# ZAX130/SmileCode

Measured on AMD Instinct MI355X. Metric: volume-pairs/sec (160x192x160) fwd+bwd, higher is better.
Workload: dtype f32; 1 GPU; ModeT 160x192x160 fp32, batch=1/GPU, full train step NCC+Grad3d fwd+bwd+Adam-amsgrad; global_batch=1, parallelism=dp1, allreduce=one flat all-reduce after backward

## Files before the change

smilecode_amd/csrc/conv3d_bf16.hip:

```cpp
#include "common.h"
#include "step_ctx.h"
#include "conv3d_internal.h"
#include <mutex>
#include <vector>

namespace {

typedef __attribute__((ext_vector_type(8))) __bf16 bf16x8;
typedef float f32x4 __attribute__((ext_vector_type(4)));
constexpr int NTHR = 256;
constexpr int TX = 16, HX = TX + 2;

__device__ __forceinline__ unsigned pack_bf16x2(float a, float b) {
  const __bf16 x = (__bf16)a, y = (__bf16)b;
  return (unsigned)__builtin_bit_cast(unsigned short, x) | ((unsigned)__builtin_bit_cast(unsigned short, y) << 16);
}
__device__ __forceinline__ unsigned short to_bf16(float a) {
  const __bf16 x = (__bf16)a;
  return __builtin_bit_cast(unsigned short, x);
}
__device__ __forceinline__ float bf16_to_f32(unsigned short u) { return __uint_as_float((unsigned)u << 16); }
__device__ __forceinline__ void split3(float x, unsigned short& hi, unsigned short& mid, unsigned short& lo) {
  hi = to_bf16(x);
  const float r1 = x - bf16_to_f32(hi);
// ... 494 lines not shown
        float4* slot = reinterpret_cast<float4*>(red + (U * 3 * NTB + n) * 256) + lane;
        float4 v = make_float4(accb[n][0], accb[n][1], accb[n][2], accb[n][3]);
        if (w4 > 0) { const float4 o = *slot; v.x += o.x; v.y += o.y; v.z += o.z; v.w += o.w; }
        *slot = v;
      }
    }
  }
  __syncthreads();
  float* out = part + ((size_t)blockIdx.x * gridDim.y + blockIdx.y) * RED_FL;
  for (int i = tid; i < RED_FL; i += NTHR) out[i] = red[i];
}

__host__ __device__ inline int colsum_rg(int gx) { return gx >= 512 ? 16 : (gx >= 256 ? 8 : (gx >= 128 ? 4 : (gx >= 64 ? 2 : 1))); }
__host__ __device__ inline int colsum_blocks(int64_t row_fl, int gx) { return (int)cdiv64(row_fl / 4, 256 / colsum_rg(gx)); }
__device__ __forceinline__ void wgrad_bf16_colsum_body(const float* __restrict__ part, float* __restrict__ red, int gx,
                                                       int64_t row_fl, int blk, double (*sm)[4]) {
  const int RG = colsum_rg(gx), QPB = 256 / RG;
  const int q = threadIdx.x % QPB, rg = threadIdx.x / QPB;
  const int64_t j = ((int64_t)blk * QPB + q) * 4;
  double a0 = 0.0, a1 = 0.0, a2 = 0.0, a3 = 0.0;
  if (j < row_fl) {
    const float* base = part + j;
    int g = rg;
    for (; g + 7 * RG < gx; g += 8 * RG) {
      float4 r[8];
#pragma unroll
      for (int u = 0; u < 8; ++u) r[u] = *reinterpret_cast<const float4*>(base + (int64_t)(g + RG * u) * row_fl);
#pragma unroll
      for (int u = 0; u < 8; ++u) asm volatile("" : "+v"(r[u].x), "+v"(r[u].y), "+v"(r[u].z), "+v"(r[u].w));
#pragma unroll
      for (int u = 0; u < 8; ++u) { a0 += (double)r[u].x; a1 += (double)r[u].y; a2 += (double)r[u].z; a3 += (double)r[u].w; }
    }
    {
      float4 r[8];
#pragma unroll
      for (int u = 0; u < 8; ++u) r[u] = *reinterpret_cast<const float4*>(base + (int64_t)(g + RG * u < gx ? g + RG * u : 0) * row_fl);
#pragma unroll
      for (int u = 0; u < 8; ++u) asm volatile("" : "+v"(r[u].x), "+v"(r[u].y), "+v"(r[u].z), "+v"(r[u].w));
#pragma unroll
      for (int u = 0; u < 8; ++u) {
        const bool in = g + RG * u < gx;
        a0 += in ? (double)r[u].x : 0.0; a1 += in ? (double)r[u].y : 0.0; a2 += in ? (double)r[u].z : 0.0; a3 += in ? (double)r[u].w : 0.0;
      }
    }
  }
  if (RG > 1) {
    sm[threadIdx.x][0] = a0; sm[threadIdx.x][1] = a1; sm[threadIdx.x][2] = a2; sm[threadIdx.x][3] = a3;
    __syncthreads();
    if (rg == 0) {
      for (int k = 1; k < RG; ++k) { a0 += sm[k * QPB + q][0]; a1 += sm[k * QPB + q][1]; a2 += sm[k * QPB + q][2]; a3 += sm[k * QPB + q][3]; }
    }
  }
  if (rg == 0 && j < row_fl) *reinterpret_cast<float4*>(red + j) = make_float4((float)a0, (float)a1, (float)a2, (float)a3);
}
__global__ __launch_bounds__(256) void wgrad_bf16_colsum_kernel(const float* __restrict__ part, float* __restrict__ red,
                                                                int gx, int64_t row_fl) {
  __shared__ double sm[256][4];
  wgrad_bf16_colsum_body(part, red, gx, row_fl, blockIdx.x, sm);
}

__device__ __forceinline__ void wgrad_bf16_reduce_body(const float* __restrict__ part, float* __restrict__ dw,
                                                       float* __restrict__ dbias, int Cin, int Cout, int CIB, int U, int NTB,
                                                       int gx, int gy, int n_coblk, int blk, int layout = 0) {
  const int nW = Cout * Cin * 27;
  const int i = blk * 256 + threadIdx.x;
  if (i >= nW + Cout) return;
  if (layout == 1) {
    const int RED_FL = (U * 2 + 1) * 256;
    int co, slot, m, q = 0;
    if (i < nW) {
      const int tap = i % 27, ci = (i / 27) % Cin;
      co = i / (27 * Cin);
      const int combo = tap / 3, dx = tap % 3;
      const int gl = CIB == 8 ? combo / 2 : combo / 4;
      m = CIB == 8 ? (combo % 2) * 8 + ci : (combo % 4) * 4 + ci;
      slot = gl * 2 + (dx == 2 ? 1 : 0);
      q = dx == 0 ? 1 : 0;
    } else {
      co = i - nW; slot = U * 2; m = 0;
    }
    const int n = q * 8 + co, lane = (m / 4) * 16 + n, reg = m % 4;
    const size_t off = (size_t)slot * 256 + lane * 4 + reg;
    double a = 0.0;
    for (int g = 0; g < gx; ++g) a += (double)part[(size_t)g * RED_FL + off];
    if (i < nW) dw[i] = (float)a;
    else if (dbias) dbias[co] = (float)a;
    return;
  }
  if (layout == 2) {
    const int NQ = CIB, MT = U, NT = NTB;
    const int RED_FL = (MT + 1) * NT * 256;
    int co, by_ci = 0, mt, c = 0, e = 0;
    if (i < nW) {
      const int tap = i % 27, ci = (i / 27) % Cin;
      co = i / (27 * Cin);
      by_ci = ci / (4 * NQ);
      const int q = (tap / 3) * NQ + (ci % (4 * NQ)) / 4;
      mt = (q >> 2) * 3 + tap % 3; c = q & 3; e = ci & 3;
    } else {
      co = i - nW; mt = MT;
    }
    const int cob = co / (16 * NT), nt = (co / 16) % NT, j = co % 16;
    const size_t off = (size_t)(by_ci * n_coblk + cob) * RED_FL + (size_t)(mt * NT + nt) * 256 + (c * 16 + j) * 4 + e;
    double a = 0.0;
    for (int g = 0; g < gx; ++g) a += (double)part[(size_t)g * gy * RED_FL + off];
    if (i < nW) dw[i] = (float)a;
    else if (dbias) dbias[co] = (float)a;
    return;
  }
  const int SLOTS = U * 3 + 1, RED_FL = SLOTS * NTB * 256;
  const int GPB = CIB == 16 ? 9 : (CIB == 8 ? 5 : 3);
  int co, slot, m, chunk;
  if (i < nW) {
    const int tap = i % 27, ci = (i / 27) % Cin;
    co = i / (27 * Cin);
    const int combo = tap / 3, dx = tap % 3;
    int gl;
    if (CIB == 16) { gl = combo; m = ci % 16; }
    else if (CIB == 8) { gl = combo / 2; m = (combo % 2) * 8 + ci; }
    else { gl = combo / 4; m = (combo % 4) * 4 + ci; }
    const int gg = (CIB == 16 ? (ci / 16) * GPB : 0) + gl;
    chunk = gg / U;
    slot = (gg % U) * 3 + dx;
  } else {
    co = i - nW; chunk = 0; slot = U * 3; m = 0;
  }
  const int nbg = co / 16, yb = nbg / NTB, nb = nbg % NTB, n = co % 16;
  const int lane = (m / 4) * 16 + n, reg = m % 4;
  const size_t off = (size_t)(chunk * n_coblk + yb) * RED_FL + (size_t)(slot * NTB + nb) * 256 + lane * 4 + reg;
  double a = 0.0;
  for (int g = 0; g < gx; ++g) a += (double)part[(size_t)g * gy * RED_FL + off];
  if (i < nW) dw[i] = (float)a;
  else if (dbias) dbias[co] = (float)a;
}
__global__ __launch_bounds__(256) void wgrad_bf16_reduce_kernel(const float* __restrict__ part, float* __restrict__ dw,
                                                                float* __restrict__ dbias, int Cin, int Cout, int CIB, int U,
                                                                int NTB, int gx, int gy, int n_coblk, int layout) {
  wgrad_bf16_reduce_body(part, dw, dbias, Cin, Cout, CIB, U, NTB, gx, gy, n_coblk, blockIdx.x, layout);
}

constexpr int BRED_MAX_JOBS = 24;
struct BRedTable { BRedJob job[BRED_MAX_JOBS]; int first[BRED_MAX_JOBS + 1]; int n; };
__global__ __launch_bounds__(256) void wgrad_bf16_colsum_many_kernel(const BRedTable t) {
  __shared__ double sm[256][4];
  int j = 0;
  while (j + 1 < t.n && (int)blockIdx.x >= t.first[j + 1]) ++j;
  const BRedJob& J = t.job[j];
  wgrad_bf16_colsum_body(J.part, J.red, J.gx, J.row_fl, blockIdx.x - t.first[j], sm);
}
__global__ __launch_bounds__(256) void wgrad_bf16_reduce_many_kernel(const BRedTable t) {
  int j = 0;
  while (j + 1 < t.n && (int)blockIdx.x >= t.first[j + 1]) ++j;
  const BRedJob& J = t.job[j];
  wgrad_bf16_reduce_body(J.red, J.dw, J.dbias, J.Cin, J.Cout, J.cib, J.u, J.ntb, 1, J.gy, J.n_coblk, blockIdx.x - t.first[j], J.layout);
}

struct WgBf16Plan { int cib, u, ntb, tz, ty, n_chunk, n_coblk, gy, gx, ntiles, tiles_x, tiles_y, tiles_z, red_fl; };
inline WgBf16Plan plan_wgrad_bf16(int B, int D, int H, int W, int Cin, int Cout) {
  WgBf16Plan p;
  if (Cin <= 4) { p.cib = 4; p.u = 3; p.ntb = 1; p.tz = 4; p.ty = 8; }
  else if (Cin <= 8) { p.cib = 8; p.u = 5; p.ntb = 1; p.tz = 4; p.ty = 8; }
  else if (Cout <= 16) { p.cib = 16; p.u = 9; p.ntb = 1; p.tz = 2; p.ty = 8; }
  else { p.cib = 16; p.u = 3; p.ntb = 2; p.tz = 2; p.ty = 4; }
  const int gpb = p.cib == 16 ? 9 : (p.cib == 8 ? 5 : 3);
  const int nblk = p.cib == 16 ? cdiv(Cin, 16) : 1;
  p.n_chunk = nblk * gpb / p.u;
  p.n_coblk = cdiv(Cout, p.ntb * 16);
  p.gy = p.n_chunk * p.n_coblk;
  p.tiles_x = cdiv(W, WTX); p.tiles_y = cdiv(H, p.ty); p.tiles_z = cdiv(D, p.tz);
  p.ntiles = B * p.tiles_x * p.tiles_y * p.tiles_z;
  int gx = (256 * 2) / p.gy;
  if (gx < 1) gx = 1;
  if (gx > p.ntiles) gx = p.ntiles;
  p.gx = gx;
  p.red_fl = (p.u * 3 + 1) * p.ntb * 256;
  return p;
}

struct Bf16Plan { int tz, ty, ck, nt, nstage, cinp, coutp, ksteps; };
inline int round_up_i(int a, int b) { return (a + b - 1) / b * b; }
inline Bf16Plan plan_tiled(int64_t V, int Cin, int Cout, int sp) {
  Bf16Plan p;
  p.cinp = round_up_i(Cin, 8);
  p.ck = (sp == 1 && p.cinp % 32 == 0) ? 32 : (p.cinp % 16 == 0 ? 16 : 8);
  p.nstage = p.cinp / p.ck;
  p.nt = Cout <= 16 ? 1 : 2;
  p.coutp = round_up_i(Cout, p.nt * 16);
  p.ksteps = (27 * p.ck + 31) / 32;
  if (V >= 60000) { p.tz = (sp == 3 && p.ck == 16) ? 2 : 4; p.ty = 8; }
  else { p.tz = 2; p.ty = 4; }
  return p;
}
inline int tiled_tiles_per_sample(int D, int H, int W, const Bf16Plan& p) { return cdiv(W, TX) * cdiv(H, p.ty) * cdiv(D, p.tz); }

inline size_t bf16_wpk_elems(int Cin, int Cout) {
  return (size_t)28 * round_up_i(Cin, 32) * round_up_i(Cout, 32) + 1024;
}

inline void launch_shift(bool x_bf16, const void* x, const float* w, const float* bias, float* shift, int B, int D, int H, int W,
                         int Cin, int Cout, hipStream_t s) {
  if (x_bf16) hipLaunchKernelGGL(conv_shift_bf16_kernel<true>, dim3(cdiv(B * Cout, 4)), dim3(256), 0, s, x, w, bias, shift, B, D, H, W, Cin, Cout);
  else hipLaunchKernelGGL(conv_shift_bf16_kernel<false>, dim3(cdiv(B * Cout, 4)), dim3(256), 0, s, x, w, bias, shift, B, D, H, W, Cin, Cout);
}

template <bool IN_BF16, bool OUT_BF16, bool STATS, int SP>
int launch_tiled(modet_step_ctx* step, const void* x, const float* w, const float* bias, void* y, void* ws, float* stats, int B,
                 int D, int H, int W, int Cin, int Cout, int mode, hipStream_t s) {
  const Bf16Plan p = plan_tiled((int64_t)D * H * W, Cin, Cout, SP);
  const unsigned short* wpk = prepacked_bf16_or_record(step, PackBKey{w, Cin, Cout, p.coutp, p.ck, p.nstage, p.ksteps, mode, SP, 0});
  const int total = p.nstage * p.ksteps * p.coutp * 32;
  if (!wpk) {
    hipLaunchKernelGGL(pack_weights_bf16_kernel, dim3(cdiv(total, 256) > 1024 ? 1024 : cdiv(total, 256)), dim3(256), 0, s, w,
                       (unsigned short*)ws, Cin, Cout, p.coutp, p.ck, p.nstage, p.ksteps, mode, SP);
    wpk = (const unsigned short*)ws;
  }
  const int wpiece = SP == 3 ? total / 8 : 0;
  const int tiles_x = cdiv(W, TX), tiles_y = cdiv(H, p.ty);
  const dim3 grid(tiled_tiles_per_sample(D, H, W, p), p.coutp / (p.nt * 16), B);
  float* rows = nullptr;
  if (STATS) {
    launch_shift(IN_BF16, x, w, bias, stats, B, D, H, W, Cin, Cout, s);
    rows = stats + (size_t)B * Cout;
  }
#define T_LAUNCH(TZ_, TY_, CK_, NT_)                                                                                       \
  hipLaunchKernelGGL((conv3d_bf16_kernel<TZ_, TY_, CK_, NT_, IN_BF16, OUT_BF16, STATS, SP>), grid, dim3(NTHR), 0, s, x,     \
                     (const uint4*)wpk, bias, y, rows, (const float*)stats, D, H, W, Cin, Cout, p.coutp, p.nstage, tiles_x, \
                     tiles_y, wpiece)
#define T_NT(TZ_, TY_, CK_) do { if (p.nt == 1) T_LAUNCH(TZ_, TY_, CK_, 1); else T_LAUNCH(TZ_, TY_, CK_, 2); } while (0)
  const int cfg = p.tz * 1000 + p.ty * 100 + p.ck;
  if (cfg == 2408) T_NT(2, 4, 8);
  else if (cfg == 2416) T_NT(2, 4, 16);
  else if (cfg == 4808) T_NT(4, 8, 8);
  else if constexpr (SP == 1) {
    if (cfg == 2432) T_NT(2, 4, 32);
    else if (cfg == 4816) T_NT(4, 8, 16);
    else if (cfg == 4832) T_NT(4, 8, 32);
    else return MODET_ERR_UNSUPPORTED;
  } else {
    if (cfg == 2816) T_NT(2, 8, 16);
    else return MODET_ERR_UNSUPPORTED;
  }
#undef T_NT
#undef T_LAUNCH
  return modet_launch_status();
}

int reduce_partials(modet_step_ctx* defer, const BRedJob& j, hipStream_t s) {
  if (defer) {
    std::lock_guard<std::mutex> lk(defer->mu);
    defer->brjobs.push_back(j);
    return modet_launch_status();
  }
  hipLaunchKernelGGL(wgrad_bf16_colsum_kernel, dim3(colsum_blocks(j.row_fl, j.gx)), dim3(256), 0, s, j.part, j.red, j.gx, j.row_fl);
  hipLaunchKernelGGL(wgrad_bf16_reduce_kernel, dim3(cdiv(j.Cout * j.Cin * 27 + j.Cout, 256)), dim3(256), 0, s, (const float*)j.red,
                     j.dw, j.dbias, j.Cin, j.Cout, j.cib, j.u, j.ntb, 1, j.gy, j.n_coblk, j.layout);
  return modet_launch_status();
}

ConvFamily route_conv16(int B, int D, int H, int W, int Cin, int Cout, int x_bf16) {
  return conv_x3_on() && modetx_x3_bf16_eligible(B, D, H, W, Cin, Cout, x_bf16) ? FAM_X3 : FAM_SPLIT;
}
ConvFamily route_wgrad16(int B, int D, int H, int W, int Cin, int Cout) {
  return conv_x3_on() && modetx_x3_bf16_wgrad_eligible(B, D, H, W, Cin, Cout) ? FAM_X3 : FAM_SPLIT;
}

}

bool modetx_split_eligible(int Cin, int Cout) { return Cin > 1 && Cin % 4 == 0 && Cout % 4 == 0; }
size_t modetx_split_ws_bytes(int Cin, int Cout) {
  const int m = Cin > Cout ? Cin : Cout;
  return 3 * bf16_wpk_elems(m, m) * sizeof(unsigned short);
}
size_t modetx_split_stats_bytes(int B, int D, int H, int W, int Cin, int Cout) {
  const size_t tiles = tiled_tiles_per_sample(D, H, W, plan_tiled((int64_t)D * H * W, Cin, Cout, 3));
  return ((size_t)B * Cout + (size_t)B * tiles * Cout * 2) * sizeof(float);
}
int modetx_split_conv(modet_step_ctx* step, const float* x, const float* w, const float* bias, float* y, void* ws, float* stats,
                      int B, int D, int H, int W, int Cin, int Cout, int mode, hipStream_t s) {
  return stats ? launch_tiled<false, false, true, 3>(step, x, w, bias, y, ws, stats, B, D, H, W, Cin, Cout, mode, s)
               : launch_tiled<false, false, false, 3>(step, x, w, bias, y, ws, nullptr, B, D, H, W, Cin, Cout, mode, s);
}

int modetx_wgrad_partials_reduce(modet_step_ctx* defer, const float* part, float* red, float* dw, float* db, int gx, int Cin,
                                 int Cout, int cib, int u, int layout, hipStream_t s) {
  const int64_t row_fl = (u * (layout == 1 ? 2 : 3) + 1) * 256;
  return reduce_partials(defer, BRedJob{part, red, dw, db, row_fl, gx, Cin, Cout, cib, u, 1, 1, 1, layout}, s);
}

int modetx_wgrad_partials_reduce2(modet_step_ctx* defer, const float* part, float* red, float* dw, float* db, int gx, int gy,
                                  int Cin, int Cout, int nq, int mt, int nt, int n_coblk, hipStream_t s) {
  const int64_t row_fl = (int64_t)gy * (mt + 1) * nt * 256;
  return reduce_partials(defer, BRedJob{part, red, dw, db, row_fl, gx, Cin, Cout, nq, mt, nt, gy, n_coblk, 2}, s);
}

void modetx_bf16_defer_flush(modet_step_ctx* c, hipStream_t stream) {
  std::vector<BRedJob> jobs;
  {
    std::lock_guard<std::mutex> lk(c->mu);
    jobs.swap(c->brjobs);
  }
  for (size_t i0 = 0; i0 < jobs.size(); i0 += BRED_MAX_JOBS) {
    BRedTable t;
    const int n = (int)(jobs.size() - i0 < (size_t)BRED_MAX_JOBS ? jobs.size() - i0 : (size_t)BRED_MAX_JOBS);
    t.n = n;
    int total = 0;
    for (int i = 0; i < n; ++i) { t.job[i] = jobs[i0 + i]; t.first[i] = total; total += colsum_blocks(t.job[i].row_fl, t.job[i].gx); }
    for (int i = n; i <= BRED_MAX_JOBS; ++i) t.first[i] = total;
    hipLaunchKernelGGL(wgrad_bf16_colsum_many_kernel, dim3(total), dim3(256), 0, stream, t);
    total = 0;
    for (int i = 0; i < n; ++i) { t.first[i] = total; total += cdiv(t.job[i].Cout * t.job[i].Cin * 27 + t.job[i].Cout, 256); }
    for (int i = n; i <= BRED_MAX_JOBS; ++i) t.first[i] = total;
    hipLaunchKernelGGL(wgrad_bf16_reduce_many_kernel, dim3(total), dim3(256), 0, stream, t);
  }
}

size_t modetx_bf16_prepack_bytes(modet_step_ctx* c) {
  std::lock_guard<std::mutex> lk(c->mu);
  size_t n = 0;
  for (const PackBKey& k : c->bjobs) n += packb_elems(k);
  return n * sizeof(unsigned short);
}
void modetx_bf16_prepack_begin(modet_step_ctx* c, void* arena, hipStream_t stream) {
  std::vector<PackBKey> jobs;
  std::vector<size_t> off;
  {
    std::lock_guard<std::mutex> lk(c->mu);
    if (c->bjobs.empty()) return;
    c->boff.assign(c->bjobs.size(), 0);
    size_t n = 0;
    for (size_t i = 0; i < c->bjobs.size(); ++i) { c->boff[i] = n; n += packb_elems(c->bjobs[i]); }
    c->barena = (unsigned short*)arena;
    for (size_t i = 0; i < c->bjobs.size(); ++i)
      if (c->bjobs[i].layout < 2) { jobs.push_back(c->bjobs[i]); off.push_back(c->boff[i]); }
  }
  for (size_t i0 = 0; i0 < jobs.size(); i0 += PACKB_MAX_JOBS) {
    PackBTable t;
    const int n = (int)(jobs.size() - i0 < (size_t)PACKB_MAX_JOBS ? jobs.size() - i0 : (size_t)PACKB_MAX_JOBS);
    int most = 1;
    for (int i = 0; i < n; ++i) {
      const PackBKey& k = jobs[i0 + i];
      t.job[i] = PackBJob{k.w, (unsigned short*)arena + off[i0 + i], k.Cin, k.Cout, k.CoutP, k.CK, k.nstage, k.ksteps, k.mode, k.npiece};
      const int blocks = cdiv(k.nstage * k.ksteps * k.CoutP * 32, 256);
      most = blocks > most ? blocks : most;
    }
    t.n = n;
    hipLaunchKernelGGL(pack_weights_bf16_many_kernel, dim3(most > 64 ? 64 : most, n), dim3(256), 0, stream, t);
  }
  modetx_x3_prepack_begin(c, stream);
}

extern "C" {

int modet_conv3d_bf16_kernel_family(int B, int D, int H, int W, int Cin, int Cout, int pass, int x_bf16) {
  if (pass == 2) return route_wgrad16(B, D, H, W, Cin, Cout);
  return pass == 1 ? route_conv16(B, D, H, W, Cout, Cin, 1) : route_conv16(B, D, H, W, Cin, Cout, x_bf16);
}

size_t modet_conv3d_bf16_ws_bytes(int Cin, int Cout) {
  const int m = Cin > Cout ? Cin : Cout;
  return bf16_wpk_elems(m, m) * sizeof(unsigned short);
}

size_t modet_conv3d_bf16_stats_bytes(int B, int D, int H, int W, int Cin, int Cout) {
  if (Cout % 4 != 0 || Cout > 128) return 0;
  const int rows = route_conv16(B, D, H, W, Cin, Cout, 0) == FAM_X3 ? modetx_x3_bf16_rows_per_sample(B, D, H, W, Cin, Cout)
                                                                   : tiled_tiles_per_sample(D, H, W, plan_tiled((int64_t)D * H * W, Cin, Cout, 1));
  return ((size_t)B * Cout + (size_t)B * (rows + 64) * Cout * 2) * sizeof(float);
}

int modet_conv3d_bf16_fwd(const void* x, int x_bf16, const float* w, const float* bias, void* y, void* ws, size_t ws_bytes,
                          float* stats, size_t stats_bytes, int B, int D, int H, int W, int Cin, int Cout,
                          modet_stream_t stream, modet_step_ctx_t* step) {
  MODET_CHECK_PTR(x); MODET_CHECK_PTR(w); MODET_CHECK_PTR(y); MODET_CHECK_PTR(ws);
  MODET_CHECK_DIM(B > 0 && D > 0 && H > 0 && W > 0 && Cin > 0 && Cout > 0 && B <= 65535);
  if (Cout % 8 != 0 || (x_bf16 ? Cin % 8 != 0 : Cin % 4 != 0)) return MODET_ERR_UNSUPPORTED;
  if (ws_bytes < bf16_wpk_elems(Cin, Cout) * sizeof(unsigned short)) return MODET_ERR_WORKSPACE;
  hipStream_t s = (hipStream_t)stream;
  if (stats && (stats_bytes < modet_conv3d_bf16_stats_bytes(B, D, H, W, Cin, Cout) || stats_bytes == 0)) return MODET_ERR_WORKSPACE;
  if (route_conv16(B, D, H, W, Cin, Cout, x_bf16) == FAM_X3) {
    if (stats) launch_shift(x_bf16, x, w, bias, stats, B, D, H, W, Cin, Cout, s);
    return modetx_x3_bf16_conv(step, x, x_bf16, w, bias, y, 1, ws, stats, B, D, H, W, Cin, Cout, 0, s);
  }
  if (stats) {
    return x_bf16 ? launch_tiled<true, true, true, 1>(step, x, w, bias, y, ws, stats, B, D, H, W, Cin, Cout, 0, s)
                  : launch_tiled<false, true, true, 1>(step, x, w, bias, y, ws, stats, B, D, H, W, Cin, Cout, 0, s);
  }
  return x_bf16 ? launch_tiled<true, true, false, 1>(step, x, w, bias, y, ws, nullptr, B, D, H, W, Cin, Cout, 0, s)
                : launch_tiled<false, true, false, 1>(step, x, w, bias, y, ws, nullptr, B, D, H, W, Cin, Cout, 0, s);
}

int modet_conv3d_bf16_bwd_data(const void* d_y, const float* w, void* d_x, int dx_bf16, void* ws, size_t ws_bytes, int B, int D,
                               int H, int W, int Cin, int Cout, modet_stream_t stream, modet_step_ctx_t* step) {
  MODET_CHECK_PTR(d_y); MODET_CHECK_PTR(w); MODET_CHECK_PTR(d_x); MODET_CHECK_PTR(ws);
  MODET_CHECK_DIM(B > 0 && D > 0 && H > 0 && W > 0 && Cin > 0 && Cout > 0 && B <= 65535);
  if (Cout % 8 != 0 || (dx_bf16 ? Cin % 8 != 0 : Cin % 4 != 0)) return MODET_ERR_UNSUPPORTED;
  if (ws_bytes < bf16_wpk_elems(Cout, Cin) * sizeof(unsigned short)) return MODET_ERR_WORKSPACE;
  hipStream_t s = (hipStream_t)stream;
  if (route_conv16(B, D, H, W, Cout, Cin, 1) == FAM_X3)
    return modetx_x3_bf16_conv(step, d_y, 1, w, nullptr, d_x, dx_bf16, ws, nullptr, B, D, H, W, Cout, Cin, 1, s);
  return dx_bf16 ? launch_tiled<true, true, false, 1>(step, d_y, w, nullptr, d_x, ws, nullptr, B, D, H, W, Cout, Cin, 1, s)
                 : launch_tiled<true, false, false, 1>(step, d_y, w, nullptr, d_x, ws, nullptr, B, D, H, W, Cout, Cin, 1, s);
}

size_t modet_conv3d_bf16_bwd_weight_ws_bytes(int B, int D, int H, int W, int Cin, int Cout) {
  const WgBf16Plan p = plan_wgrad_bf16(B, D, H, W, Cin, Cout);
  size_t need = ((size_t)p.gx + 1) * p.gy * p.red_fl * sizeof(float);
  if (route_wgrad16(B, D, H, W, Cin, Cout) == FAM_X3) {
    const size_t x3 = modetx_x3_bf16_wgrad_ws_bytes(B, D, H, W, Cin, Cout);
    need = x3 > need ? x3 : need;
  }
  return need;
}

static int bf16_bwd_weight_impl(const void* x, int x_bf16, const void* d_y, float* d_w, float* d_bias, void* ws,
                                size_t ws_bytes, int B, int D, int H, int W, int Cin, int Cout, modet_stream_t stream,
                                modet_step_ctx* defer);

int modet_conv3d_bf16_bwd_weight(const void* x, int x_bf16, const void* d_y, float* d_w, float* d_bias, void* ws,
                                 size_t ws_bytes, int B, int D, int H, int W, int Cin, int Cout, modet_stream_t stream) {
  return bf16_bwd_weight_impl(x, x_bf16, d_y, d_w, d_bias, ws, ws_bytes, B, D, H, W, Cin, Cout, stream, nullptr);
}
int modet_conv3d_bf16_bwd_weight_defer(const void* x, int x_bf16, const void* d_y, float* d_w, float* d_bias, void* ws,
                                       size_t ws_bytes, int B, int D, int H, int W, int Cin, int Cout, modet_stream_t stream,
                                       modet_step_ctx_t* step) {
  MODET_CHECK_PTR(step);
  return bf16_bwd_weight_impl(x, x_bf16, d_y, d_w, d_bias, ws, ws_bytes, B, D, H, W, Cin, Cout, stream, step);
}

static int bf16_bwd_weight_impl(const void* x, int x_bf16, const void* d_y, float* d_w, float* d_bias, void* ws,
                                size_t ws_bytes, int B, int D, int H, int W, int Cin, int Cout, modet_stream_t stream,
                                modet_step_ctx* defer) {
  MODET_CHECK_PTR(x); MODET_CHECK_PTR(d_y); MODET_CHECK_PTR(d_w); MODET_CHECK_PTR(ws);
  MODET_CHECK_DIM(B > 0 && D > 0 && H > 0 && W > 0 && Cin > 0 && Cout > 0);
  if (Cout % 8 != 0 || (x_bf16 ? Cin % 8 != 0 : Cin % 4 != 0)) return MODET_ERR_UNSUPPORTED;
  if (Cin > 8 && Cin % 16 != 0) return MODET_ERR_UNSUPPORTED;
  if (Cin == 4 && x_bf16) return MODET_ERR_UNSUPPORTED;
  if (ws_bytes < modet_conv3d_bf16_bwd_weight_ws_bytes(B, D, H, W, Cin, Cout)) return MODET_ERR_WORKSPACE;
  hipStream_t s = (hipStream_t)stream;
  if (route_wgrad16(B, D, H, W, Cin, Cout) == FAM_X3)
    return modetx_x3_bf16_wgrad(defer, x, x_bf16, d_y, d_w, d_bias, ws, B, D, H, W, Cin, Cout, s);
  const WgBf16Plan p = plan_wgrad_bf16(B, D, H, W, Cin, Cout);
  const dim3 grid(p.gx, p.gy);
#define WG_BF(CIB_, U_, NTB_, TZ_, TY_)                                                                                     \
  do {                                                                                                                     \
    if (x_bf16) hipLaunchKernelGGL((conv3d_bf16_wgrad_kernel<CIB_, U_, NTB_, TZ_, TY_, true>), grid, dim3(NTHR), 0, s, x,  \
                                   (const unsigned short*)d_y, (float*)ws, D, H, W, Cin, Cout, p.tiles_x, p.tiles_y, p.tiles_z, \
                                   p.ntiles, p.n_coblk);                                                                    \
    else hipLaunchKernelGGL((conv3d_bf16_wgrad_kernel<CIB_, U_, NTB_, TZ_, TY_, false>), grid, dim3(NTHR), 0, s, x,        \
                            (const unsigned short*)d_y, (float*)ws, D, H, W, Cin, Cout, p.tiles_x, p.tiles_y, p.tiles_z,    \
                            p.ntiles, p.n_coblk);                                                                           \
  } while (0)
  if (p.cib == 4) hipLaunchKernelGGL((conv3d_bf16_wgrad_kernel<4, 3, 1, 4, 8, false>), grid, dim3(NTHR), 0, s, x,
                                     (const unsigned short*)d_y, (float*)ws, D, H, W, Cin, Cout, p.tiles_x, p.tiles_y, p.tiles_z,
                                     p.ntiles, p.n_coblk);
  else if (p.cib == 8) WG_BF(8, 5, 1, 4, 8);
  else if (p.u == 9) WG_BF(16, 9, 1, 2, 8);
  else WG_BF(16, 3, 2, 2, 4);
#undef WG_BF
  const int64_t row_fl = (int64_t)p.gy * p.red_fl;
  float* red = (float*)ws + (size_t)p.gx * row_fl;
  return reduce_partials(defer, BRedJob{(const float*)ws, red, d_w, d_bias, row_fl, p.gx, Cin, Cout, p.cib, p.u, p.ntb, p.gy, p.n_coblk, 0}, s);
// ... 4 lines not shown
```

smilecode_amd/csrc/conv3d_internal.h:

```cpp
#pragma once
#include "common.h"
#include "step_ctx.h"

enum ConvFamily { FAM_EXACT = 0, FAM_SPLIT = 1, FAM_X3 = 2, FAM_DIRECT = 3, FAM_WTR = 4, FAM_Q = 5 };
inline bool conv_x3_on() { static const bool on = modet_tuning_env("MODET_CONV_X3") != '0'; return on; }

bool modetx_split_eligible(int Cin, int Cout);
size_t modetx_split_ws_bytes(int Cin, int Cout);
size_t modetx_split_stats_bytes(int B, int D, int H, int W, int Cin, int Cout);
int modetx_split_conv(modet_step_ctx* step, const float* x, const float* w, const float* bias, float* y, void* ws, float* stats,
                      int B, int D, int H, int W, int Cin, int Cout, int mode, hipStream_t s);
int modetx_wgrad_partials_reduce(modet_step_ctx* defer, const float* part, float* red, float* dw, float* db, int gx, int Cin,
                                 int Cout, int cib, int u, int layout, hipStream_t s);
int modetx_wgrad_partials_reduce2(modet_step_ctx* defer, const float* part, float* red, float* dw, float* db, int gx, int gy,
                                  int Cin, int Cout, int nq, int mt, int nt, int n_coblk, hipStream_t s);
size_t modetx_bf16_prepack_bytes(modet_step_ctx* c);
void modetx_bf16_prepack_begin(modet_step_ctx* c, void* arena, hipStream_t stream);
void modetx_bf16_defer_flush(modet_step_ctx* c, hipStream_t stream);

bool modetx_x3_eligible(int B, int D, int H, int W, int Cin, int Cout);
size_t modetx_x3_ws_bytes(int Cin, int Cout);
size_t modetx_x3_stats_bytes(int B, int D, int H, int W, int Cin, int Cout);
int modetx_x3_conv(modet_step_ctx* step, const float* x, const float* w, const float* bias, float* y, void* ws, float* stats,
                   const float* in_mean, const float* in_rstd, int B, int D, int H, int W, int Cin, int Cout, int act, int mode,
                   hipStream_t s, const float* amax = nullptr, bool x_free = false);
size_t modetx_x3_bst_rows_bytes(int B, int D, int H, int W, int Cin, int Cout);
int modetx_x3_dgrad_bst(modet_step_ctx* step, const float* dy, const float* w, float* dx, const float* xraw, const float* mean,
                        const float* rstd, float* rows, void* ws, int B, int D, int H, int W, int Cin, int Cout, hipStream_t s,
                        const float* amax = nullptr);
bool modetx_x3_wgrad_eligible(int B, int D, int H, int W, int Cin, int Cout);
size_t modetx_x3_wgrad_ws_bytes(int B, int D, int H, int W, int Cin, int Cout);
int modetx_x3_wgrad(modet_step_ctx* defer, const float* x, const float* dy, float* dw, float* db, void* ws, int B, int D, int H,
                    int W, int Cin, int Cout, hipStream_t s, const float* amax = nullptr, const float* in_mean = nullptr,
                    const float* in_rstd = nullptr);
bool modetx_x3_bf16_eligible(int B, int D, int H, int W, int Cin, int Cout, int x_bf16);
int modetx_x3_bf16_rows_per_sample(int B, int D, int H, int W, int Cin, int Cout);
int modetx_x3_bf16_conv(modet_step_ctx* step, const void* x, int x_bf16, const float* w, const float* bias, void* y, int y_bf16,
                        void* ws, float* stats, int B, int D, int H, int W, int Cin, int Cout, int mode, hipStream_t s);
bool modetx_x3_bf16_wgrad_eligible(int B, int D, int H, int W, int Cin, int Cout);
size_t modetx_x3_bf16_wgrad_ws_bytes(int B, int D, int H, int W, int Cin, int Cout);
int modetx_x3_bf16_wgrad(modet_step_ctx* defer, const void* x, int x_bf16, const void* dy, float* dw, float* db, void* ws, int B,
                         int D, int H, int W, int Cin, int Cout, hipStream_t s);
void modetx_x3_prepack_begin(modet_step_ctx* c, hipStream_t stream);

bool modetx_q_eligible(int B, int D, int H, int W, int Cin, int Cout);
size_t modetx_q_ws_bytes(int Cin, int Cout);
size_t modetx_q_stats_bytes(int B, int D, int H, int W, int Cin, int Cout);
int modetx_q_conv(modet_step_ctx* step, const float* x, const float* w, const float* bias, float* y, void* ws, float* stats,
                  const float* in_mean, const float* in_rstd, int B, int D, int H, int W, int Cin, int Cout, int mode,
                  hipStream_t s, const float* amax = nullptr, const float* xraw = nullptr, const float* bmean = nullptr,
                  const float* brstd = nullptr, float* bst_rows = nullptr, bool x_free = false);
size_t modetx_q_bst_rows_bytes(int B, int D, int H, int W, int Cin, int Cout);
void modetx_q_prepack_begin(modet_step_ctx* c, hipStream_t stream);

bool modetx_wtr_eligible(int B, int D, int H, int W, int Cin, int Cout);
size_t modetx_wtr_ws_bytes(int B, int D, int H, int W, int Cin, int Cout);
bool modetx_wtr_batches(int B, int D, int H, int W);
void modetx_wtr_flush(modet_step_ctx* c, hipStream_t s);
int modetx_wtr_wgrad(modet_step_ctx* defer, const float* x, const float* dy, float* dw, float* db, void* ws, int B, int D, int H,
                     int W, int Cin, int Cout, hipStream_t s, const float* amax = nullptr);
```

smilecode_amd/csrc/conv3d_wtr.hip:

```cpp
#include "common.h"
#include "step_ctx.h"
#include "conv3d_internal.h"

namespace {

typedef __attribute__((ext_vector_type(8))) __bf16 bf16x8;
typedef float f32x4 __attribute__((ext_vector_type(4)));
typedef short v4s __attribute__((ext_vector_type(4)));
typedef short v8s __attribute__((ext_vector_type(8)));
using u32x4 = unsigned __attribute__((ext_vector_type(4)));
using BufRsrc = __amdgpu_buffer_rsrc_t;

constexpr int NTHR = 256;
constexpr int TZ = 2, TY = 8, TX = 8, HZ = TZ + 2, HY = TY + 2, HX = TX + 2;
constexpr int HVOX = HZ * HY * HX, VOX = TZ * TY * TX;
constexpr int ROWB = 32;
constexpr int XP = 12;
constexpr int XPL = HZ * HY * XP * ROWB;
constexpr int DPL = VOX * ROWB;
constexpr unsigned WTR_OOB = 0x80000000u;

__device__ __forceinline__ BufRsrc tensor_rsrc(const float* base, unsigned bytes) {
  const uint64_t a = reinterpret_cast<uint64_t>(base);
  const uint64_t u = ((uint64_t)(unsigned)__builtin_amdgcn_readfirstlane((unsigned)(a >> 32)) << 32) |
                     (uint64_t)(unsigned)__builtin_amdgcn_readfirstlane((unsigned)a);
  return __builtin_amdgcn_make_buffer_rsrc(reinterpret_cast<void*>(u), 0, (int)__builtin_amdgcn_readfirstlane(bytes), 0x00020000);
}
__device__ __forceinline__ void split3_pk(float a, float b, unsigned& hi, unsigned& mid, unsigned& lo) {
  typedef __attribute__((ext_vector_type(2))) __bf16 bf16x2;
  typedef __attribute__((ext_vector_type(2))) float f32x2;
  auto pk = [](float u, float v) -> unsigned {
    const bf16x2 t = __builtin_convertvector((f32x2){u, v}, bf16x2);
    return __builtin_bit_cast(unsigned, t);
  };
  hi = pk(a, b);
  const float ra = a - __uint_as_float(hi << 16), rb = b - __uint_as_float(hi & 0xffff0000u);
  mid = pk(ra, rb);
  const float sa = ra - __uint_as_float(mid << 16), sb = rb - __uint_as_float(mid & 0xffff0000u);
  lo = pk(sa, sb);
}
typedef _Float16 h16x8 __attribute__((ext_vector_type(8)));
constexpr float WTR_F16_XSCALE = 16.f;
#ifndef WTR_F16
#define WTR_F16 1
#endif
__device__ __forceinline__ void split2h_pk(float a, float b, unsigned& hi, unsigned& lo) {
  typedef __attribute__((ext_vector_type(2))) _Float16 h16x2;
  typedef __attribute__((ext_vector_type(2))) float f32x2;
  const h16x2 t = __builtin_convertvector((f32x2){a, b}, h16x2);
  hi = __builtin_bit_cast(unsigned, t);
  const h16x2 r = __builtin_convertvector((f32x2){a - (float)t[0], b - (float)t[1]}, h16x2);
  lo = __builtin_bit_cast(unsigned, r);
}
template <bool F16>
__device__ __forceinline__ f32x4 wtr_mma(bf16x8 a, bf16x8 b, f32x4 c) {
  if constexpr (F16) return __builtin_amdgcn_mfma_f32_16x16x32_f16(__builtin_bit_cast(h16x8, a), __builtin_bit_cast(h16x8, b), c, 0, 0, 0);
  else return __builtin_amdgcn_mfma_f32_16x16x32_bf16(a, b, c, 0, 0, 0);
}
__device__ __forceinline__ uint2 tr_read(const unsigned char* lds, int off) {
  typedef __attribute__((address_space(3))) v4s* lptr;
  return __builtin_bit_cast(uint2, __builtin_amdgcn_ds_read_tr16_b64_v4i16((lptr)(lds + off)));
}
__device__ __forceinline__ bf16x8 frag(unsigned a, unsigned b, unsigned c, unsigned d) {
  const u32x4 v = {a, b, c, d};
  return __builtin_bit_cast(bf16x8, v);
}

#ifdef MODET_TUNING
__device__ long long* g_wtr_dbg = nullptr;
#endif

struct WtrArgs {
  const float* x; const float* dy; float* part;
  int B, D, H, W, Cin, Cout, tiles_x, tiles_y, tiles_z, ntiles, n_coblk;
  const float* amax;
};
constexpr int WTR_MAX_JOBS = 8;
struct WtrTable {
  WtrArgs job[WTR_MAX_JOBS];
  int first[WTR_MAX_JOBS + 1], gx[WTR_MAX_JOBS], gy[WTR_MAX_JOBS];
  int n;
};

#ifndef WTR_VARIANT
#define WTR_VARIANT 8
#endif
template <int NQ, int NT, bool VEC, int NP = 3>
__global__ __launch_bounds__(NTHR, 2) void conv_wgrad_tr_kernel(const WtrTable t) {
  static_assert(NP == 3 || NP == 2, "three bf16 pieces or two f16 pieces");
  int job = 0;
  while (job + 1 < t.n && (int)blockIdx.x >= t.first[job + 1]) ++job;
  const WtrArgs a = t.job[job];
  const int grid_x = t.gx[job], grid_y = t.gy[job];
  const int lb = (int)blockIdx.x - t.first[job];
  const int blk_x = lb / grid_y, blk_y = lb - blk_x * grid_y;
  constexpr int NF = (9 * NQ + 3) / 4;
  constexpr int MT = 3 * NF;
  constexpr int KS = NT;
  constexpr int XS_BYTES = NP * XPL, DS_BYTES = NP * NT * DPL;
  constexpr int RED_FL = (MT + 1) * NT * 256;
  constexpr int LDS_BYTES = XS_BYTES + DS_BYTES > RED_FL * 4 ? XS_BYTES + DS_BYTES : RED_FL * 4;
  __shared__ __attribute__((aligned(16))) unsigned char lds[LDS_BYTES];

#ifdef MODET_TUNING
  const long long t_entry = __builtin_readcyclecounter();
#endif
  const int tid = threadIdx.x, lane = tid & 63;
  const int wave = __builtin_amdgcn_readfirstlane(tid >> 6);
  const int kg = lane >> 4, S = lane & 15, sj = S >> 2, sc = S & 3;
  const int nw = NT == 2 ? (wave & 1) : 0;
  const int s_first = NT == 2 ? 2 * (wave >> 1) : wave;
  const int cib = blk_y / a.n_coblk, cob = blk_y - cib * a.n_coblk;
  const int ci0 = cib * 4 * NQ, co0 = cob * 16 * NT;
  const int D = a.D, H = a.H, W = a.W, Cin = a.Cin, Cout = a.Cout;

  int aoff[NF];
#pragma unroll
  for (int f = 0; f < NF; ++f) {
    int q = 4 * f + sc;
    if (q >= 9 * NQ) q = 0;
    const int zy = q / NQ, quad = q - zy * NQ;
    aoff[f] = ((zy / 3) * HY + zy % 3) * XP * ROWB + quad * 8;
  }
  const int abase = (((s_first >> 1) * HY + 4 * (s_first & 1) + kg) * XP + sj) * ROWB;
  const int yrow = 4 * (s_first & 1) + kg;
  const int bslot = ((s_first >> 1) * TY + yrow) * TX;
  const int bsw = (kg & 1) << 2;
  const int boff0 = XS_BYTES + nw * DPL + (bslot + (sj ^ bsw)) * ROWB + sc * 8;
  const int boff1 = XS_BYTES + nw * DPL + (bslot + ((4 + sj) ^ bsw)) * ROWB + sc * 8;
  const unsigned one2 = S == 0 ? (NP == 2 ? 0x3c003c00u : 0x3f803f80u) : 0u;
  float dsc = 1.f, dinv = 1.f;
  if constexpr (NP == 2) {
    float m = a.amax[lane * MODET_AMAX_STRIDE];
#pragma unroll
    for (int o = 32; o >= 1; o >>= 1) m = fmaxf(m, __shfl_xor(m, o, 64));
    if (m > 0.f && m < __builtin_huge_valf()) {
      int e;
      (void)frexpf(m, &e);
      int sh = 15 - e;
      sh = sh > 100 ? 100 : (sh < -100 ? -100 : sh);
      dsc = ldexpf(1.f, sh); dinv = ldexpf(1.f, -sh);
    }
  }

  f32x4 acc[NF][3], accb = {0.f, 0.f, 0.f, 0.f};
#pragma unroll
  for (int f = 0; f < NF; ++f)
#pragma unroll
    for (int d = 0; d < 3; ++d) acc[f][d] = (f32x4){0.f, 0.f, 0.f, 0.f};

  const BufRsrc rx = tensor_rsrc(a.x, (unsigned)((int64_t)a.B * D * H * W * Cin * 4));
  const BufRsrc rd = tensor_rsrc(a.dy, (unsigned)((int64_t)a.B * D * H * W * Cout * 4));

  constexpr int IPR = HX * NQ, RP = NQ >= 3 ? 5 : (NQ == 2 ? 10 : 20), NPASS = HZ * HY / RP;
  const int r_t = tid / IPR, i_t = tid - r_t * IPR;
// ... 72 lines not shown
          *reinterpret_cast<uint2*>(dst) = make_uint2(h0, h1);
          *reinterpret_cast<uint2*>(dst + XPL) = make_uint2(m0, m1);
          *reinterpret_cast<uint2*>(dst + 2 * XPL) = make_uint2(l0, l1);
        }
      }
    }
#pragma unroll
    for (int i = 0; i < NDP; ++i) {
      const int v = i * DVP + dv_t;
      const int slot = (v & ~7) | ((v & 7) ^ (((v >> 3) & 1) << 2));
      unsigned char* dst = lds + dlds_t + slot * ROWB;
      if constexpr (NP == 2) {
        unsigned h0, l0, h1, l1;
        split2h_pk(__uint_as_float(dr[i][0]) * dsc, __uint_as_float(dr[i][1]) * dsc, h0, l0);
        split2h_pk(__uint_as_float(dr[i][2]) * dsc, __uint_as_float(dr[i][3]) * dsc, h1, l1);
        *reinterpret_cast<uint2*>(dst) = make_uint2(h0, h1);
        *reinterpret_cast<uint2*>(dst + NT * DPL) = make_uint2(l0, l1);
      } else {
        unsigned h0, m0, l0, h1, m1, l1;
        split3_pk(__uint_as_float(dr[i][0]), __uint_as_float(dr[i][1]), h0, m0, l0);
        split3_pk(__uint_as_float(dr[i][2]), __uint_as_float(dr[i][3]), h1, m1, l1);
        *reinterpret_cast<uint2*>(dst) = make_uint2(h0, h1);
        *reinterpret_cast<uint2*>(dst + NT * DPL) = make_uint2(m0, m1);
        *reinterpret_cast<uint2*>(dst + 2 * NT * DPL) = make_uint2(l0, l1);
      }
    }
  };

#ifdef MODET_TUNING
  long long tph[7] = {0, 0, 0, 0, 0, 0, 0}, tq0, tq1;
#define TPH(k) do { tq1 = __builtin_readcyclecounter(); tph[k] += tq1 - tq0; tq0 = tq1; } while (0)
#else
#define TPH(k) do { } while (0)
#endif
  int tile = blk_x;
  if (!(WTR_VARIANT & 2) && tile < a.ntiles) load_tile(tile);
#ifdef MODET_TUNING
  tq0 = __builtin_readcyclecounter();
  tph[5] = tq0 - t_entry;
#endif
  for (; tile < a.ntiles; tile += grid_x) {
    if (WTR_VARIANT & 2) load_tile(tile);
    TPH(0);
    __syncthreads();
    TPH(1);
    if (WTR_VARIANT & 8) __builtin_amdgcn_s_setprio(2);
    write_tile();
    TPH(2);
    __syncthreads();
    TPH(3);
    if (!(WTR_VARIANT & 2) && tile + grid_x < a.ntiles) load_tile(tile + grid_x);
    if (WTR_VARIANT & 8) __builtin_amdgcn_s_setprio(0);
    TPH(0);
    auto load_raw = [&](int u, uint2 (&R)[NP][3]) {
      const int ks = u / NF, f = u - ks * NF;
      const int o = abase + aoff[f] + ks * 4 * XP * ROWB;
#pragma unroll
      for (int p = 0; p < NP; ++p)
#pragma unroll
        for (int b = 0; b < 3; ++b) R[p][b] = tr_read(lds, o + p * XPL + b * 4 * ROWB);
    };
    uint2 Rc[NP][3], Rn[NP][3];
    bf16x8 bq[NP];
    load_raw(0, Rc);
#pragma unroll
    for (int u = 0; u < KS * NF; ++u) {
      const int ks = u / NF, f = u - ks * NF;
      if (f == 0) {
#pragma unroll
        for (int p = 0; p < NP; ++p) {
          const uint2 lo = tr_read(lds, boff0 + p * NT * DPL + ks * 4 * TX * ROWB), hi = tr_read(lds, boff1 + p * NT * DPL + ks * 4 * TX * ROWB);
          bq[p] = frag(lo.x, lo.y, hi.x, hi.y);
        }
      }
      if (!(WTR_VARIANT & 4) && u + 1 < KS * NF) load_raw(u + 1, Rn);
      __builtin_amdgcn_sched_barrier(0);
      if (f == 0) {
        const bf16x8 on = frag(one2, one2, one2, one2);
        if constexpr (NP == 3) accb = wtr_mma<false>(on, bq[NP - 1], accb);
        accb = wtr_mma<NP == 2>(on, bq[1], accb);
        accb = wtr_mma<NP == 2>(on, bq[0], accb);
      }
      bf16x8 d0[NP], d1[NP], d2[NP];
#pragma unroll
      for (int p = 0; p < NP; ++p) {
        const unsigned r0 = Rc[p][0].x, r1 = Rc[p][0].y, r2 = Rc[p][1].x, r3 = Rc[p][1].y, r4 = Rc[p][2].x;
        d0[p] = frag(r0, r1, r2, r3);
        d2[p] = frag(r1, r2, r3, r4);
        d1[p] = frag(__builtin_amdgcn_alignbit(r1, r0, 16), __builtin_amdgcn_alignbit(r2, r1, 16),
                     __builtin_amdgcn_alignbit(r3, r2, 16), __builtin_amdgcn_alignbit(r4, r3, 16));
      }
#define MM3(PA, PB)                                                                                   \
      acc[f][0] = wtr_mma<NP == 2>(d0[PA], bq[PB], acc[f][0]);       \
      acc[f][1] = wtr_mma<NP == 2>(d1[PA], bq[PB], acc[f][1]);       \
      acc[f][2] = wtr_mma<NP == 2>(d2[PA], bq[PB], acc[f][2]);
      if constexpr (NP == 3) { MM3(NP - 1, 0) MM3(0, NP - 1) MM3(1, 1) }
      MM3(1, 0) MM3(0, 1) MM3(0, 0)
#undef MM3
      __builtin_amdgcn_sched_barrier(0);
      if (u + 1 < KS * NF) {
        if (WTR_VARIANT & 4) load_raw(u + 1, Rc);
        else {
#pragma unroll
          for (int p = 0; p < NP; ++p)
#pragma unroll
            for (int b = 0; b < 3; ++b) Rc[p][b] = Rn[p][b];
        }
      }
    }
    TPH(4);
  }
  if constexpr (NP == 2) {
    const float winv = dinv * (1.f / WTR_F16_XSCALE);
#pragma unroll
    for (int f = 0; f < NF; ++f)
#pragma unroll
      for (int d = 0; d < 3; ++d) { acc[f][d][0] *= winv; acc[f][d][1] *= winv; acc[f][d][2] *= winv; acc[f][d][3] *= winv; }
    accb[0] *= dinv; accb[1] *= dinv; accb[2] *= dinv; accb[3] *= dinv;
  }
  float* red = reinterpret_cast<float*>(lds);
  constexpr int ROUNDS = 4 / NT;
#pragma unroll 1
  for (int r = 0; r < ROUNDS; ++r) {
    __syncthreads();
    if ((NT == 2 ? (wave >> 1) : wave) == r) {
#pragma unroll
      for (int f = 0; f < NF; ++f)
#pragma unroll
        for (int d = 0; d < 3; ++d) {
          float4* slot = reinterpret_cast<float4*>(red + ((f * 3 + d) * NT + nw) * 256) + lane;
          float4 v = make_float4(acc[f][d][0], acc[f][d][1], acc[f][d][2], acc[f][d][3]);
          if (r > 0) { const float4 o = *slot; v.x += o.x; v.y += o.y; v.z += o.z; v.w += o.w; }
          *slot = v;
        }
      float4* slot = reinterpret_cast<float4*>(red + (MT * NT + nw) * 256) + lane;
      float4 v = make_float4(accb[0], accb[1], accb[2], accb[3]);
      if (r > 0) { const float4 o = *slot; v.x += o.x; v.y += o.y; v.z += o.z; v.w += o.w; }
      *slot = v;
    }
  }
  __syncthreads();
  float* out = a.part + (size_t)lb * (size_t)RED_FL;
  for (int i = tid * 4; i < RED_FL; i += NTHR * 4) *reinterpret_cast<float4*>(out + i) = *reinterpret_cast<const float4*>(red + i);
#ifdef MODET_TUNING
  TPH(6);
  if (g_wtr_dbg && lane == 0) {
    long long* o = g_wtr_dbg + ((int64_t)(blk_y * grid_x + blk_x) * 4 + wave) * 8;
    for (int i = 0; i < 7; ++i) o[i] = tph[i];
    o[7] = t_entry;
  }
#endif
}

struct WtrPlan { int nq, nt, n_cib, n_coblk, gy, gx, tiles_x, tiles_y, tiles_z, ntiles, mt, red_fl; };
inline WtrPlan wtr_plan(int B, int D, int H, int W, int Cin, int Cout) {
  WtrPlan p;
  const int quads = (Cin + 3) / 4;
  p.nq = quads % 4 == 0 ? 4 : (quads % 3 == 0 ? 3 : (quads % 2 == 0 ? 2 : 1));
  p.n_cib = quads / p.nq;
  p.nt = Cout > 16 ? 2 : 1;
  p.n_coblk = cdiv(Cout, 16 * p.nt);
  p.gy = p.n_cib * p.n_coblk;
  p.tiles_x = cdiv(W, TX); p.tiles_y = cdiv(H, TY); p.tiles_z = cdiv(D, TZ);
  p.ntiles = B * p.tiles_x * p.tiles_y * p.tiles_z;
  int slots = 512;
  if (const char e = modet_tuning_env("MODET_WTR_SLOTS")) slots = e == '1' ? 256 : (e == '2' ? 384 : 512);
  int gx = slots / p.gy;
  if (gx < 1) gx = 1;
  if (gx > p.ntiles) gx = p.ntiles;
  p.gx = gx;
  p.mt = 3 * ((9 * p.nq + 3) / 4);
  p.red_fl = (p.mt + 1) * p.nt * 256;
  return p;
}

}

#ifdef MODET_TUNING
extern "C" int modet_debug_wtr_timing(long long* buf) {
  return (int)hipMemcpyToSymbol(HIP_SYMBOL(g_wtr_dbg), &buf, sizeof(buf));
}
#endif

bool modetx_wtr_eligible(int B, int D, int H, int W, int Cin, int Cout) {
  const int64_t n = (int64_t)B * D * H * W;
  const bool vec = Cin % 4 == 0 && Cout % 4 == 0;
  return Cin >= 4 && n * (Cin > Cout ? Cin : Cout) * 4 < 0x7fffffffLL && Cout <= 256 && Cin <= 1024 && (vec || Cout <= 16);
}
size_t modetx_wtr_ws_bytes(int B, int D, int H, int W, int Cin, int Cout) {
  const WtrPlan p = wtr_plan(B, D, H, W, Cin, Cout);
  const int gx = p.gy >= 512 ? 1 : 512 / p.gy;
  return ((size_t)gx + 1) * p.gy * p.red_fl * sizeof(float);
}
static void wtr_launch(const WtrTable& t, int nq, int nt, bool vec, bool f16, hipStream_t s) {
  const dim3 grid(t.first[t.n]);
#define WTR_L(NQ_, NT_, V_, NP_) hipLaunchKernelGGL((conv_wgrad_tr_kernel<NQ_, NT_, V_, NP_>), grid, dim3(NTHR), 0, s, t)
#define WTR_Q(NT_, V_, NP_) do { if (nq == 4) WTR_L(4, NT_, V_, NP_); else if (nq == 3) WTR_L(3, NT_, V_, NP_); else if (nq == 2) WTR_L(2, NT_, V_, NP_); else WTR_L(1, NT_, V_, NP_); } while (0)
#define WTR_P(NP_) do { \
    if (nt == 2) WTR_Q(2, true, NP_);                   \
    else if (vec) WTR_Q(1, true, NP_); \
    else WTR_Q(1, false, NP_); } while (0)
  if (f16) WTR_P(2); else WTR_P(3);
#undef WTR_P
#undef WTR_Q
#undef WTR_L
}

#ifndef WTR_BATCH_MAX_VOXELS
#define WTR_BATCH_MAX_VOXELS 1500000
#endif
bool modetx_wtr_batches(int B, int D, int H, int W) { return (int64_t)B * D * H * W <= WTR_BATCH_MAX_VOXELS; }

int modetx_wtr_wgrad(modet_step_ctx* defer, const float* x, const float* dy, float* dw, float* db, void* ws, int B, int D, int H,
                     int W, int Cin, int Cout, hipStream_t s, const float* amax) {
  const WtrPlan p = wtr_plan(B, D, H, W, Cin, Cout);
  const bool vec = Cin % 4 == 0 && Cout % 4 == 0;
  if (!WTR_F16 || (int64_t)D * H * W >= (1ll << 24)) amax = nullptr;
  float* red = (float*)ws + (size_t)p.gx * p.gy * p.red_fl;
  if (defer && modetx_wtr_batches(B, D, H, W)) {
    WtrQueued j{x, dy, (float*)ws, B, D, H, W, Cin, Cout, p.tiles_x, p.tiles_y, p.tiles_z, p.ntiles, p.n_coblk, p.nq, p.nt, vec ? 1 : 0,
                p.gx, p.gy, amax};
    {
      std::lock_guard<std::mutex> lk(defer->mu);
      defer->wtrjobs.push_back(j);
    }
    return modetx_wgrad_partials_reduce2(defer, (const float*)ws, red, dw, db, p.gx, p.gy, Cin, Cout, p.nq, p.mt, p.nt, p.n_coblk, s);
  }
  WtrTable t;
  t.job[0] = WtrArgs{x, dy, (float*)ws, B, D, H, W, Cin, Cout, p.tiles_x, p.tiles_y, p.tiles_z, p.ntiles, p.n_coblk, amax};
  t.first[0] = 0; t.first[1] = p.gx * p.gy; t.gx[0] = p.gx; t.gy[0] = p.gy; t.n = 1;
  wtr_launch(t, p.nq, p.nt, vec, amax != nullptr, s);
  return modetx_wgrad_partials_reduce2(defer, (const float*)ws, red, dw, db, p.gx, p.gy, Cin, Cout, p.nq, p.mt, p.nt, p.n_coblk, s);
}

void modetx_wtr_flush(modet_step_ctx* c, hipStream_t s) {
  std::vector<WtrQueued> jobs;
  {
    std::lock_guard<std::mutex> lk(c->mu);
    jobs.swap(c->wtrjobs);
  }
  std::vector<char> done(jobs.size(), 0);
  for (size_t i = 0; i < jobs.size(); ++i) {
    if (done[i]) continue;
    WtrTable t;
    t.n = 0; t.first[0] = 0;
    for (size_t k = i; k < jobs.size() && t.n < WTR_MAX_JOBS; ++k) {
      const WtrQueued& q = jobs[k];
      if (done[k] || q.nq != jobs[i].nq || q.nt != jobs[i].nt || q.vec != jobs[i].vec || (q.amax != nullptr) != (jobs[i].amax != nullptr)) continue;
      t.job[t.n] = WtrArgs{q.x, q.dy, q.part, q.B, q.D, q.H, q.W, q.Cin, q.Cout, q.tiles_x, q.tiles_y, q.tiles_z, q.ntiles, q.n_coblk, q.amax};
      t.gx[t.n] = q.gx; t.gy[t.n] = q.gy;
      t.first[t.n + 1] = t.first[t.n] + q.gx * q.gy;
      ++t.n;
      done[k] = 1;
    }
    for (int k = t.n; k < WTR_MAX_JOBS; ++k) { t.first[k + 1] = t.first[t.n]; t.gx[k] = 1; t.gy[k] = 1; }
    wtr_launch(t, jobs[i].nq, jobs[i].nt, jobs[i].vec != 0, jobs[i].amax != nullptr, s);
  }
}
```

Before: 142.6 volume-pairs/sec.

## Cap WTR split-K rows and skip colsum pass when one partial row

```diff
diff --git a/smilecode_amd/csrc/conv3d_bf16.hip b/smilecode_amd/csrc/conv3d_bf16.hip
--- a/smilecode_amd/csrc/conv3d_bf16.hip
+++ b/smilecode_amd/csrc/conv3d_bf16.hip
@@ -670,7 +670,9 @@
   int j = 0;
   while (j + 1 < t.n && (int)blockIdx.x >= t.first[j + 1]) ++j;
   const BRedJob& J = t.job[j];
-  wgrad_bf16_reduce_body(J.red, J.dw, J.dbias, J.Cin, J.Cout, J.cib, J.u, J.ntb, 1, J.gy, J.n_coblk, blockIdx.x - t.first[j], J.layout);
+  const bool direct = modetx_wgrad_reduce_direct(J.gx, J.layout);
+  wgrad_bf16_reduce_body(direct ? J.part : J.red, J.dw, J.dbias, J.Cin, J.Cout, J.cib, J.u, J.ntb, direct ? J.gx : 1, J.gy, J.n_coblk,
+                         blockIdx.x - t.first[j], J.layout);
 }
 
 struct WgBf16Plan { int cib, u, ntb, tz, ty, n_chunk, n_coblk, gy, gx, ntiles, tiles_x, tiles_y, tiles_z, red_fl; };
@@ -769,9 +771,11 @@
     defer->brjobs.push_back(j);
     return modet_launch_status();
   }
-  hipLaunchKernelGGL(wgrad_bf16_colsum_kernel, dim3(colsum_blocks(j.row_fl, j.gx)), dim3(256), 0, s, j.part, j.red, j.gx, j.row_fl);
-  hipLaunchKernelGGL(wgrad_bf16_reduce_kernel, dim3(cdiv(j.Cout * j.Cin * 27 + j.Cout, 256)), dim3(256), 0, s, (const float*)j.red,
-                     j.dw, j.dbias, j.Cin, j.Cout, j.cib, j.u, j.ntb, 1, j.gy, j.n_coblk, j.layout);
+  const bool direct = modetx_wgrad_reduce_direct(j.gx, j.layout);
+  if (!direct) hipLaunchKernelGGL(wgrad_bf16_colsum_kernel, dim3(colsum_blocks(j.row_fl, j.gx)), dim3(256), 0, s, j.part, j.red, j.gx, j.row_fl);
+  hipLaunchKernelGGL(wgrad_bf16_reduce_kernel, dim3(cdiv(j.Cout * j.Cin * 27 + j.Cout, 256)), dim3(256), 0, s,
+                     direct ? j.part : (const float*)j.red, j.dw, j.dbias, j.Cin, j.Cout, j.cib, j.u, j.ntb, direct ? j.gx : 1, j.gy,
+                     j.n_coblk, j.layout);
   return modet_launch_status();
 }
 
@@ -822,9 +826,12 @@
     const int n = (int)(jobs.size() - i0 < (size_t)BRED_MAX_JOBS ? jobs.size() - i0 : (size_t)BRED_MAX_JOBS);
     t.n = n;
     int total = 0;
-    for (int i = 0; i < n; ++i) { t.job[i] = jobs[i0 + i]; t.first[i] = total; total += colsum_blocks(t.job[i].row_fl, t.job[i].gx); }
+    for (int i = 0; i < n; ++i) {
+      t.job[i] = jobs[i0 + i]; t.first[i] = total;
+      if (!modetx_wgrad_reduce_direct(t.job[i].gx, t.job[i].layout)) total += colsum_blocks(t.job[i].row_fl, t.job[i].gx);
+    }
     for (int i = n; i <= BRED_MAX_JOBS; ++i) t.first[i] = total;
-    hipLaunchKernelGGL(wgrad_bf16_colsum_many_kernel, dim3(total), dim3(256), 0, stream, t);
+    if (total > 0) hipLaunchKernelGGL(wgrad_bf16_colsum_many_kernel, dim3(total), dim3(256), 0, stream, t);
     total = 0;
     for (int i = 0; i < n; ++i) { t.first[i] = total; total += cdiv(t.job[i].Cout * t.job[i].Cin * 27 + t.job[i].Cout, 256); }
     for (int i = n; i <= BRED_MAX_JOBS; ++i) t.first[i] = total;
diff --git a/smilecode_amd/csrc/conv3d_internal.h b/smilecode_amd/csrc/conv3d_internal.h
--- a/smilecode_amd/csrc/conv3d_internal.h
+++ b/smilecode_amd/csrc/conv3d_internal.h
@@ -14,6 +14,10 @@
                                  int Cout, int cib, int u, int layout, hipStream_t s);
 int modetx_wgrad_partials_reduce2(modet_step_ctx* defer, const float* part, float* red, float* dw, float* db, int gx, int gy,
                                   int Cin, int Cout, int nq, int mt, int nt, int n_coblk, hipStream_t s);
+#ifndef WGRAD_DIRECT_MAX_ROWS
+#define WGRAD_DIRECT_MAX_ROWS 1
+#endif
+__host__ __device__ inline bool modetx_wgrad_reduce_direct(int gx, int layout) { return layout == 2 && gx <= WGRAD_DIRECT_MAX_ROWS; }
 size_t modetx_bf16_prepack_bytes(modet_step_ctx* c);
 void modetx_bf16_prepack_begin(modet_step_ctx* c, void* arena, hipStream_t stream);
 void modetx_bf16_defer_flush(modet_step_ctx* c, hipStream_t stream);
diff --git a/smilecode_amd/csrc/conv3d_wtr.hip b/smilecode_amd/csrc/conv3d_wtr.hip
--- a/smilecode_amd/csrc/conv3d_wtr.hip
+++ b/smilecode_amd/csrc/conv3d_wtr.hip
@@ -1,6 +1,8 @@
 #include "common.h"
 #include "step_ctx.h"
 #include "conv3d_internal.h"
+
+#include <algorithm>
 
 namespace {
 
@@ -379,6 +381,9 @@
 #endif
 }
 
+#ifndef WTR_ROW_TILES
+#define WTR_ROW_TILES 5
+#endif
 struct WtrPlan { int nq, nt, n_cib, n_coblk, gy, gx, tiles_x, tiles_y, tiles_z, ntiles, mt, red_fl; };
 inline WtrPlan wtr_plan(int B, int D, int H, int W, int Cin, int Cout) {
   WtrPlan p;
@@ -394,6 +399,9 @@
   if (const char e = modet_tuning_env("MODET_WTR_SLOTS")) slots = e == '1' ? 256 : (e == '2' ? 384 : 512);
   int gx = slots / p.gy;
   if (gx < 1) gx = 1;
+  int want = p.ntiles / WTR_ROW_TILES;
+  if (want < 1) want = 1;
+  if (gx > want) gx = want;
   if (gx > p.ntiles) gx = p.ntiles;
   p.gx = gx;
   p.mt = 3 * ((9 * p.nq + 3) / 4);
@@ -408,6 +416,14 @@
   return (int)hipMemcpyToSymbol(HIP_SYMBOL(g_wtr_dbg), &buf, sizeof(buf));
 }
 #endif
+
+extern "C" int modet_debug_wtr_plan(int B, int D, int H, int W, int Cin, int Cout, int* out) {
+  if (!out || B < 1 || D < 1 || H < 1 || W < 1 || Cin < 1 || Cout < 1) return -1;
+  const WtrPlan p = wtr_plan(B, D, H, W, Cin, Cout);
+  const int v[8] = {p.gx, p.gy, p.ntiles, p.red_fl, modetx_wgrad_reduce_direct(p.gx, 2) ? 1 : 0, WTR_ROW_TILES, p.nq, p.nt};
+  for (int i = 0; i < 8; ++i) out[i] = v[i];
+  return 0;
+}
 
 bool modetx_wtr_eligible(int B, int D, int H, int W, int Cin, int Cout) {
   const int64_t n = (int64_t)B * D * H * W;
@@ -466,6 +482,7 @@
     std::lock_guard<std::mutex> lk(c->mu);
     jobs.swap(c->wtrjobs);
   }
+  std::stable_sort(jobs.begin(), jobs.end(), [](const WtrQueued& a, const WtrQueued& b) { return cdiv(a.ntiles, a.gx) > cdiv(b.ntiles, b.gx); });
   std::vector<char> done(jobs.size(), 0);
   for (size_t i = 0; i < jobs.size(); ++i) {
     if (done[i]) continue;
```

Result: no change. 143.4 volume-pairs/sec (median of 6 runs) (+0.6%).
